# metaverse3d2022/Nerf-Cuda

Hardware: AMD Instinct MI355X
Metric: megasamples/s (march samples composited into a ray = the reference's per-ray sample count), Lego-like NeRF render @1920x1080 (higher is better)
Workload: dtype f16

## Files before the change

nerf-cuda_amd/csrc/nrf_api.hip:

```cpp

#include <hip/hip_runtime.h>

#include <chrono>
#include <cmath>
#include <cstdio>
#include <cstdlib>
#include <cstring>
#include <limits>
#include <mutex>
#include <string>
#include <vector>

#include "nrf_device.h"
#include "nrf_generic.h"
#include "nrf_launch.h"

using namespace nrf;

namespace {

thread_local std::string g_err;
int fail(int code, const std::string& msg) {
  g_err = msg;
  return code;
// ... 338 lines not shown
        const uint32_t res = Lv.res;
        Lv.q_off_b = far ? (uint32_t)(end_bytes >> 4) : (uint32_t)end_bytes;
        Lv.q_my_b = far ? res : res << 4;
        Lv.q_mz_b = far ? res * res : (res * res) << 4;
        Lv.q_max = res - 1;
        end_bytes += (uint64_t)res * res * (res + 1) * 16;
      }
    }
    p.table_bytes = end_bytes;
  }
  const uint32_t sh_b = F == 8 ? 4u : (F == 4 ? 3u : (F == 1 ? 1u : 2u));
  for (LevelParams& Lv : p.lp) {
    const bool hashed_pow2 = Lv.mode == LV_HASH_POW2;
    Lv.off_b = Lv.offset << sh_b;
    if (hashed_pow2) {
      Lv.my_b = 2654435761u << sh_b;
      Lv.mz_b = 805459861u << sh_b;
    } else {
      Lv.my_b = (Lv.my_b >> 2) << sh_b;
      Lv.mz_b = (Lv.mz_b >> 2) << sh_b;
    }
    Lv.mask_b = (hashed_pow2 || Lv.mode == LV_ADD_POW2) ? ((Lv.size - 1) << sh_b) : 0xffffffffu;
  }
  return p;
}

void nerf_matrix_to_ngp(const float p[16], float s, float R[9], float org[3]) {
  const int rows[3] = {1, 2, 0};
  for (int r = 0; r < 3; ++r) {
    const float* src = p + 4 * rows[r];
    R[3 * r + 0] = src[0];
    R[3 * r + 1] = -src[1];
    R[3 * r + 2] = -src[2];
    org[r] = src[3] * s + 0.0f;
  }
}

}

struct nrf_context {
  int device = 0;
  hipStream_t stream = nullptr;
  hipEvent_t ev0 = nullptr, ev1 = nullptr;
  bool model_loaded = false;
  nrf_model_desc desc{};
  nrf_level_table lv{};
  DevModel dm{};
  void* d_grid = nullptr;
  void* d_occ = nullptr;
  void* d_wfrag = nullptr;
  void* d_lv = nullptr;
  void* d_coarse = nullptr;
  void* d_dilated = nullptr;
  void* d_ctab = nullptr;
  void* d_gen = nullptr;
  void* d_wfrag_gen = nullptr;
  bool rays_persistent = false;
  int own_net = NET_HOT;
  void* d_wfrag_hot = nullptr;
  GenModel gen{};
  std::vector<float> host_grid;
  bool grid_missing = false;
  bool allow_persistent = true;
  bool centre_out = true;
  bool allow_gen_wlds = true;
  bool allow_width_instances = true;
  int queue_classes = 0;
  int n_cus = 256;
  nrf_options opt{};
  int W = 0, H = 0;
  int n_local_tiles = 0;
  int max_views = 1;
  int last_views = 1;
  size_t n_out_px = 0;
  size_t n_alloc_px = 0;
  void* d_rgba = nullptr;
  void* d_depth = nullptr;
  void* d_plan = nullptr;
  int plan_max_pos = 1 << 14;
  void* d_counters = nullptr;
  int call_index = 0;
  int quad_levels = -1;
  int quad_budget_mb = -1;
  uint64_t table_bytes = 0, table_ref_bytes = 0;
  uint32_t gather_addresses = 0;
  bool allow_gen_fast_grid = true;
  int march_ff = 1;
  int tail_split = 1;
  void* d_rgb8 = nullptr;
  void* d_depth8 = nullptr;
  void* bound_rgba = nullptr;
  void* bound_depth = nullptr;
  void* bound_rgbd8 = nullptr;
  void* bound_rgb8 = nullptr;
  void* bound_depth8 = nullptr;
  struct HostSlot {
    void* d_buf = nullptr;
    uint8_t* h_buf = nullptr;
    size_t views = 0, px = 0;
    hipEvent_t done = nullptr, t0 = nullptr, t1 = nullptr;
    hipEvent_t grp[2] = {nullptr, nullptr};
    std::vector<int> row_lo, row_hi;
    std::vector<int> col_lo, col_hi;
    int bg = -1;
    int n_views = 0, W = 0, H = 0;
    bool with_depth = true, pending = false;
    uint64_t copied = 0;
    std::vector<int> rows;
    unsigned* d_done = nullptr;
    unsigned* h_flags = nullptr;
    size_t prog_entries = 0;
    unsigned epoch = 0;
    bool progressive = false, copies_issued = false;
  } hs[2];
  int hs_next = 0;
  hipStream_t copy_stream = nullptr;
  bool host_merge = true;
  bool host_progressive = true;
  bool host_cols = true;
  bool host_skip_outside = true;
  void* last_rgba = nullptr;
  void* last_depth = nullptr;
  int march_budget = 256;
  bool sample_cap_forced = false;
  int sample_cap = 2;
  bool rendered = false;
  hipStream_t last_stream = nullptr;
};

namespace {

int set_device(nrf_context* c) {
  HIP_TRY(hipSetDevice(c->device));
  return NRF_OK;
}

void free_model(nrf_context* c) {
  if (c->d_grid) (void)hipFree(c->d_grid);
  if (c->d_occ) (void)hipFree(c->d_occ);
  if (c->d_wfrag) (void)hipFree(c->d_wfrag);
  if (c->d_lv) (void)hipFree(c->d_lv);
  if (c->d_coarse) (void)hipFree(c->d_coarse);
  if (c->d_ctab) (void)hipFree(c->d_ctab);
  if (c->d_dilated) (void)hipFree(c->d_dilated);
  if (c->d_gen) (void)hipFree(c->d_gen);
  if (c->d_wfrag_gen) (void)hipFree(c->d_wfrag_gen);
  if (c->d_wfrag_hot) (void)hipFree(c->d_wfrag_hot);
  c->d_wfrag_gen = c->d_wfrag_hot = nullptr;
  c->d_grid = c->d_occ = c->d_wfrag = c->d_lv = c->d_coarse = c->d_ctab = c->d_dilated = c->d_gen = nullptr;
  c->model_loaded = false;
}

constexpr int CALL_RING = 16;
constexpr size_t CALL_SLOT_BYTES = COUNTER_BYTES + 128 + 65536;
constexpr int HOST_SLOTS = 2;
constexpr uint32_t QUAD_BUDGET_MB_DEFAULT = 8192;
inline char* call_slot(const nrf_context* c, int index) { return (char*)c->d_counters + (size_t)(index % CALL_RING) * CALL_SLOT_BYTES; }

void free_host_slots(nrf_context* c) {
  for (auto& h : c->hs) {
    if (h.d_buf) (void)hipFree(h.d_buf);
    if (h.h_buf) (void)hipHostFree(h.h_buf);
    if (h.d_done) (void)hipFree(h.d_done);
    if (h.h_flags) (void)hipHostFree(h.h_flags);
    h.d_buf = nullptr;
    h.h_buf = nullptr;
    h.d_done = h.h_flags = nullptr;
    h.views = h.px = h.prog_entries = 0;
    h.bg = -1;
    h.pending = false;
  }
}

void free_frame(nrf_context* c) {
  if (c->d_rgba) (void)hipFree(c->d_rgba);
  if (c->d_depth) (void)hipFree(c->d_depth);
  if (c->d_rgb8) (void)hipFree(c->d_rgb8);
  if (c->d_depth8) (void)hipFree(c->d_depth8);
  c->d_rgba = c->d_depth = c->d_rgb8 = c->d_depth8 = nullptr;
  c->n_out_px = 0;
  c->rendered = false;
}

int total_strips(int W, int H) { return ((((W + 7) / 8) + 3) / 4) * ((H + 7) / 8); }

int local_tiles(int W, int H, int shard_index, int shard_count) {
  const int total = total_strips(W, H);
  if (shard_index >= total) return 0;
  return 4 * ((total - shard_index + shard_count - 1) / shard_count);
}

bool tiled_layout(const nrf_context* c) { return c->opt.shard_count > 1 || c->opt.tile_major != 0; }

int alloc_frame(nrf_context* c) {
  if (c->W <= 0 || c->H <= 0) return NRF_OK;
  const bool tiled = tiled_layout(c);
  c->n_local_tiles = local_tiles(c->W, c->H, c->opt.shard_index, c->opt.shard_count);
  int tps = 0;
  nrf_tiles_per_shard(c->W, c->H, c->opt.shard_count, &tps);
  const size_t per_view = tiled ? (size_t)tps * 64 : (size_t)c->W * c->H;
  const size_t need = per_view * (size_t)c->max_views;
  if (per_view == c->n_out_px && need == c->n_alloc_px && c->d_rgba) return NRF_OK;
  HIP_TRY(hipDeviceSynchronize());
  free_frame(c);
  HIP_TRY(hipMalloc(&c->d_rgba, need * 16));
  HIP_TRY(hipMalloc(&c->d_depth, need * 4));
  HIP_TRY(hipMemsetAsync(c->d_rgba, 0, need * 16, c->stream));
  HIP_TRY(hipMemsetAsync(c->d_depth, 0, need * 4, c->stream));
  HIP_TRY(hipStreamSynchronize(c->stream));
  c->n_out_px = per_view;
  c->n_alloc_px = need;
  return NRF_OK;
}

int fill_frame_params(nrf_context* c, const float cam[4], const float pose[16], FrameParams& P) {
  std::memset(&P, 0, sizeof(P));
  nerf_matrix_to_ngp(pose, c->desc.scale, P.R, P.org);
  for (int i = 0; i < 4; ++i) P.cam[i] = cam[i];
  P.W = c->W;
  P.H = c->H;
  P.tiles_x = (c->W + 7) / 8;
  P.tiles_y = (c->H + 7) / 8;
  P.shard_index = c->opt.shard_index;
  P.shard_count = c->opt.shard_count;
  P.n_local_tiles = c->n_local_tiles;
  P.tile_major = tiled_layout(c);
  P.bg_color = c->opt.bg_color;
  P.min_near = c->opt.min_near;
  P.dt_gamma = c->opt.dt_gamma;
  P.density_scale = c->opt.density_scale;
  P.max_steps = c->opt.max_steps;
  P.march_budget = c->march_budget;
  P.sample_cap = c->sample_cap;
  P.centre_out = c->centre_out ? 1 : 0;
  P.out_mode = c->bound_rgbd8 ? OUT_RGBD8 : (c->bound_rgb8 ? OUT_U8 : OUT_F32);
  P.skip_outside = 0;
  P.prog_done = P.prog_flags = nullptr;
  P.prog_epoch = 0;
  P.tail_split = c->tail_split;
  P.perturb = c->opt.perturb;
  P.march_ff = c->opt.perturb ? 0 : c->march_ff;
  P.fast_interp = c->opt.fast_interp ? 1 : 0;
  P.queue_classes = c->queue_classes;
  return NRF_OK;
}

void view_roi(const float R[9], const float org[3], const float cam[4], const float box[6], int W, int H, int roi[4]) {
  roi[0] = 0; roi[1] = 0; roi[2] = W - 1; roi[3] = H - 1;
  if (!(box[0] <= box[3])) {
    roi[2] = -1;
    roi[3] = -1;
    return;
  }
  const double a = R[0], b = R[1], cc = R[2], d = R[3], e = R[4], f = R[5], g = R[6], h = R[7], i = R[8];
  const double det = a * (e * i - f * h) - b * (d * i - f * g) + cc * (d * h - e * g);
  if (!(std::fabs(det) > 1e-12)) return;
  const double inv[9] = {(e * i - f * h) / det, (cc * h - b * i) / det, (b * f - cc * e) / det,
                         (f * g - d * i) / det, (a * i - cc * g) / det, (cc * d - a * f) / det,
                         (d * h - e * g) / det, (b * g - a * h) / det, (a * e - b * d) / det};
  double lo[2] = {1e300, 1e300}, hi[2] = {-1e300, -1e300};
  for (int c = 0; c < 8; ++c) {
    const double p[3] = {(double)box[(c & 1) ? 3 : 0] - org[0], (double)box[(c & 2) ? 4 : 1] - org[1],
                         (double)box[(c & 4) ? 5 : 2] - org[2]};
    const double vx = inv[0] * p[0] + inv[1] * p[1] + inv[2] * p[2];
    const double vy = inv[3] * p[0] + inv[4] * p[1] + inv[5] * p[2];
    const double vz = inv[6] * p[0] + inv[7] * p[1] + inv[8] * p[2];
    if (!(vz > 1e-3)) return;
    const double u = cam[2] + cam[0] * vx / vz, v = cam[3] + cam[1] * vy / vz;
    if (!(u == u) || !(v == v)) return;
    lo[0] = u < lo[0] ? u : lo[0]; hi[0] = u > hi[0] ? u : hi[0];
    lo[1] = v < lo[1] ? v : lo[1]; hi[1] = v > hi[1] ? v : hi[1];
  }
  const double m = 3.0;
  const double x0 = std::floor(lo[0] - 0.5 - m), y0 = std::floor(lo[1] - 0.5 - m);
  const double x1 = std::ceil(hi[0] - 0.5 + m), y1 = std::ceil(hi[1] - 0.5 + m);
  roi[0] = x0 < 0 ? 0 : (x0 > W ? W : (int)x0);
  roi[1] = y0 < 0 ? 0 : (y0 > H ? H : (int)y0);
  roi[2] = x1 < -1 ? -1 : (x1 > W - 1 ? W - 1 : (int)x1);
  roi[3] = y1 < -1 ? -1 : (y1 > H - 1 ? H - 1 : (int)y1);
}

int set_density_grid(nrf_context* c, const float* density_grid, float mean_density) {
  const nrf_model_desc* d = &c->desc;
  const uint64_t Hh = d->density_grid_size;
  const uint64_t cells = Hh * Hh * Hh * d->cascade;
  HIP_TRY(hipDeviceSynchronize());
  for (void** q : {&c->d_occ, &c->d_coarse, &c->d_ctab, &c->d_dilated}) {
    if (*q) (void)hipFree(*q);
    *q = nullptr;
  }
  const float thresh = fminf(0.01f, mean_density);
  std::vector<uint32_t> occ((cells + 31) / 32 + 1, 0u);
  for (uint64_t i = 0; i < cells; ++i)
    if (density_grid[i] > thresh) occ[i >> 5] |= 1u << (i & 31);

  const uint32_t Hs = d->density_grid_size, Cs = d->cascade;
  const uint32_t coarse_shift = (Hs % 4 == 0 && Hs >= 8) ? 2u : 0u;
  std::vector<uint32_t> coarse;
  if (coarse_shift) {
    const uint32_t Hc = Hs >> 2;
    coarse.assign(((uint64_t)Cs * Hc * Hc * Hc + 31) / 32 + 1, 0u);
    for (uint64_t i = 0; i < cells; ++i) {
      if (!((occ[i >> 5] >> (i & 31)) & 1u)) continue;
      const uint32_t level = (uint32_t)(i / (Hh * Hh * Hh));
      const uint64_t r = i % (Hh * Hh * Hh);
      const uint32_t nx = (uint32_t)(r / (Hh * Hh)), ny = (uint32_t)((r / Hh) % Hh), nz = (uint32_t)(r % Hh);
      const uint64_t cc = (((uint64_t)level * Hc + (nx >> 2)) * Hc + (ny >> 2)) * Hc + (nz >> 2);
      coarse[cc >> 5] |= 1u << (cc & 31);
    }
  }
  auto reachable = [&](uint32_t level, uint32_t nx, uint32_t ny, uint32_t nz) {
    if (level == 0 || Cs <= 1) return true;
    const double mb = fmin(ldexp(1.0, (int)level), (double)d->bound), cell = 2.0 * mb / (double)Hs;
    const uint32_t n3[3] = {nx, ny, nz};
    double r_max = 0.0;
    for (int a = 0; a < 3; ++a) {
      const double lo = -mb + n3[a] * cell, hi = lo + cell;
      r_max = fmax(r_max, fmax(fabs(lo), fabs(hi)));
    }
    return !(r_max + cell < ldexp(1.0, (int)level - 1));
  };
  float occ_box[6] = {1.f, 1.f, 1.f, -1.f, -1.f, -1.f};
  bool boundary_occupied = false;
  {
    bool any = false;
    for (uint32_t level = 0; level < Cs; ++level) {
      uint32_t lo[3] = {Hs, Hs, Hs}, hi[3] = {0, 0, 0};
      bool lvl_any = false;
      for (uint64_t r = 0; r < Hh * Hh * Hh; ++r) {
        const uint64_t i = (uint64_t)level * Hh * Hh * Hh + r;
        if (!((occ[i >> 5] >> (i & 31)) & 1u)) continue;
        const uint32_t n3[3] = {(uint32_t)(r / (Hh * Hh)), (uint32_t)((r / Hh) % Hh), (uint32_t)(r % Hh)};
        if (!reachable(level, n3[0], n3[1], n3[2])) continue;
        for (int a = 0; a < 3; ++a) { lo[a] = n3[a] < lo[a] ? n3[a] : lo[a]; hi[a] = n3[a] > hi[a] ? n3[a] : hi[a]; }
        lvl_any = true;
      }
      if (!lvl_any) continue;
      const double mip_bound = fmin(Cs > 1 ? ldexp(1.0, (int)level) : 1.0, (double)d->bound);
      const double cell = 2.0 * mip_bound / (double)Hs;
      for (int a = 0; a < 3; ++a) {
        float wlo = (float)(-mip_bound + ((double)lo[a] - 2.0) * cell);
        float whi = (float)(-mip_bound + ((double)hi[a] + 3.0) * cell);
        if (lo[a] == 0) wlo = fminf(wlo, fminf(d->aabb[a], -d->bound) - (float)(2.0 * cell));
        if (hi[a] == Hs - 1) whi = fmaxf(whi, fmaxf(d->aabb[a + 3], d->bound) + (float)(2.0 * cell));
        if (!any || wlo < occ_box[a]) occ_box[a] = wlo;
        if (!any || whi > occ_box[a + 3]) occ_box[a + 3] = whi;
        boundary_occupied = boundary_occupied || lo[a] == 0 || hi[a] == Hs - 1;
      }
      any = true;
    }
  }
  bool exterior_positions = false;
  {
    const float outer = fminf(Cs > 1 ? ldexpf(1.0f, (int)Cs - 1) : 1.0f, d->bound);
    exterior_positions = d->bound > outer;
    for (int a = 0; a < 3; ++a) exterior_positions = exterior_positions || d->aabb[a] < -d->bound || d->aabb[a + 3] > d->bound;
  }
  const bool visibility_walk = !(exterior_positions && boundary_occupied);
  std::vector<uint32_t> dilated;
  uint32_t dilated_level_words = 0;
  if (coarse_shift && visibility_walk) {
    const int Hc = (int)(Hs >> 2), Hf = (int)Hs;
    dilated_level_words = (uint32_t)(((uint64_t)Hc * Hc * Hc + 31) / 32);
    dilated.assign((size_t)dilated_level_words * Cs, 0u);
    for (uint32_t level = 0; level < Cs; ++level) {
      uint32_t* dl = dilated.data() + (size_t)level * dilated_level_words;
      for (int x = 0; x < Hf; ++x)
        for (int y = 0; y < Hf; ++y)
          for (int z = 0; z < Hf; ++z) {
            const uint64_t i = (((uint64_t)level * Hf + x) * Hf + y) * Hf + z;
            if (!((occ[i >> 5] >> (i & 31)) & 1u)) continue;
            if (!reachable(level, (uint32_t)x, (uint32_t)y, (uint32_t)z)) continue;
            for (int dx = -1; dx <= 1; ++dx)
              for (int dy = -1; dy <= 1; ++dy)
                for (int dz = -1; dz <= 1; ++dz) {
                  const int X = x + dx, Y = y + dy, Z = z + dz;
                  if (X < 0 || Y < 0 || Z < 0 || X >= Hf || Y >= Hf || Z >= Hf) continue;
                  const uint64_t nn = ((uint64_t)(X >> 2) * Hc + (Y >> 2)) * Hc + (Z >> 2);
                  dl[nn >> 5] |= 1u << (nn & 31);
                }
          }
    }
  }
  std::vector<float> ctab((size_t)Cs * (Hs + 1));
  for (uint32_t level = 0; level < Cs; ++level) {
    const float mip_bound = fminf(Cs > 1 ? ldexpf(1.0f, (int)level) : 1.0f, d->bound);
    const float Hm1 = (float)(Hs - 1);
    for (uint32_t v = 0; v <= Hs; ++v) ctab[(size_t)level * (Hs + 1) + v] = ((float)v / Hm1 * 2 - 1) * mip_bound;
  }

  auto upload = [&](void** dst, const void* src, size_t bytes) -> hipError_t {
    hipError_t e = hipMalloc(dst, bytes);
    if (e != hipSuccess) return e;
    return hipMemcpyAsync(*dst, src, bytes, hipMemcpyHostToDevice, c->stream);
  };
  HIP_TRY(upload(&c->d_occ, occ.data(), occ.size() * 4));
  if (coarse_shift) HIP_TRY(upload(&c->d_coarse, coarse.data(), coarse.size() * 4));
  HIP_TRY(upload(&c->d_ctab, ctab.data(), ctab.size() * 4));
  if (!dilated.empty()) HIP_TRY(upload(&c->d_dilated, dilated.data(), dilated.size() * 4));
  HIP_TRY(hipStreamSynchronize(c->stream));
  HIP_TRY(hipDeviceSynchronize());
  DevModel& M = c->dm;
  M.occ_bits = (const uint32_t*)c->d_occ;
  for (int i = 0; i < 6; ++i) M.occ_box[i] = occ_box[i];
  M.occ_coarse = (const uint32_t*)c->d_coarse;
  M.cell_bound = (const float*)c->d_ctab;
  M.occ_dilated = (const uint32_t*)c->d_dilated;
  M.coarse_shift = coarse_shift;
  M.lds_coarse_words = M.lds_ctab_floats = M.lds_dilated_words = 0;
  {
    const uint64_t words = coarse_shift ? (uint64_t)coarse.size() : 0, fl = ctab.size();
    uint64_t budget = (uint64_t)render_lds_table_max_bytes();
    if (M.stage == NET_GENERIC) {
      const uint64_t used = (uint64_t)render_gen_lds_fixed_bytes(M.gen_wave_bytes);
      budget = used + budget <= 160u * 1024u ? budget : 160u * 1024u - used;
    }
    if (M.stage == NET_WIDE) {
      const uint64_t room = 160u * 1024u / 3u - (uint64_t)render_wide_lds_fixed_bytes();
      budget = budget < room ? budget : room;
    }
    if (coarse_shift && 4 * (words + fl) <= budget) {
      M.lds_coarse_words = (uint32_t)words;
      M.lds_ctab_floats = (uint32_t)fl;
    }
  }
  M.dilated_level_words = dilated_level_words;
  if (!dilated.empty() && dilated.size() * 4 <= (size_t)N_FRAGS * 64 * 16) M.lds_dilated_words = (uint32_t)dilated.size();
  M.net = M.stage;
  M.persistent = 0;
  M.persist_waves = 0;
  M.gen_weights_lds = 0;
  M.n_cus = (uint32_t)c->n_cus;
  if (c->allow_persistent && M.lds_coarse_words > 0) {
    const size_t tables = 4 * ((size_t)M.lds_coarse_words + M.lds_ctab_floats + dilated.size());
    const int form = march_form(M.H, M.cascade, M.bound);
    for (const int net : {c->own_net, (int)M.stage}) {
      const int first_waves = render_persist_waves(net, form);
      for (int waves : {first_waves, net == NET_GENERIC && first_waves != 8 ? 8 : 0}) {
        if (waves == 0 || M.persistent) break;
        const size_t fixed = (size_t)render_persistent_lds_bytes(net, waves, M.gen_wave_bytes) + tables;
        for (int wlds : {1, 0}) {
          if (wlds && (net != NET_GENERIC || !c->allow_gen_wlds)) continue;
          if (fixed + (wlds ? 16u + M.gen_frag_bytes : 0u) <= 160u * 1024u) {
            M.net = (uint32_t)net;
            M.persistent = 1;
            M.persist_waves = (uint32_t)waves;
            M.gen_weights_lds = (uint32_t)wlds;
            M.lds_dilated_words = (uint32_t)dilated.size();
            break;
          }
        }
      }
      if (M.persistent) break;
    }
  }
  c->rays_persistent = M.persistent != 0 && M.net == NET_HOT;
  c->desc.mean_density = mean_density;
  c->host_grid.assign(density_grid, density_grid + cells);
  return NRF_OK;
}
// ... 48 lines not shown

int nrf_tiles_per_shard(int width, int height, int shard_count, int* n) {
  if (!n || width <= 0 || height <= 0 || shard_count <= 0) return fail(NRF_E_INVALID, "bad argument");
  *n = 4 * ((total_strips(width, height) + shard_count - 1) / shard_count);
  return NRF_OK;
}

int nrf_create(int device, nrf_context** out) {
  if (!out) return fail(NRF_E_INVALID, "null argument");
  int count = 0;
  hipError_t e = hipGetDeviceCount(&count);
  if (e != hipSuccess || count <= 0)
    return fail(NRF_E_NODEVICE, "no HIP device available (this library has no CPU fallback)");
  if (device < 0 || device >= count) return fail(NRF_E_NODEVICE, "device index out of range");
  hipDeviceProp_t prop;
  HIP_TRY(hipGetDeviceProperties(&prop, device));
  if (std::strncmp(prop.gcnArchName, "gfx950", 6) != 0)
    return fail(NRF_E_NODEVICE, std::string("device is ") + prop.gcnArchName + ", this library is built for gfx950 only");
  nrf_context* c = new nrf_context;
  c->device = device;
  nrf_default_options(&c->opt);
  if (const char* e = std::getenv("NRF_MARCH_BUDGET")) {
    const int b = std::atoi(e);
    if (b >= 1 && b <= 4096) c->march_budget = b;
  }
  if (const char* e = std::getenv("NRF_SAMPLE_CAP")) { c->sample_cap = std::atoi(e); c->sample_cap_forced = true; }
  if (const char* e = std::getenv("NRF_PERSISTENT")) c->allow_persistent = std::atoi(e) != 0;
  if (const char* e = std::getenv("NRF_CENTRE_OUT")) c->centre_out = std::atoi(e) != 0;
  if (const char* e = std::getenv("NRF_GEN_WLDS")) c->allow_gen_wlds = std::atoi(e) != 0;
  if (const char* e = std::getenv("NRF_WIDTH_INSTANCES")) c->allow_width_instances = std::atoi(e) != 0;
  if (const char* e = std::getenv("NRF_QUEUE_CLASSES")) c->queue_classes = std::atoi(e);
  c->n_cus = prop.multiProcessorCount > 0 ? prop.multiProcessorCount : 256;
  HIP_TRY(hipSetDevice(device));
  HIP_TRY(hipStreamCreateWithFlags(&c->stream, hipStreamNonBlocking));
  HIP_TRY(hipEventCreate(&c->ev0));
  HIP_TRY(hipEventCreate(&c->ev1));
  if (const char* e = std::getenv("NRF_HOST_PROGRESSIVE")) c->host_progressive = std::atoi(e) != 0;
  if (const char* e = std::getenv("NRF_HOST_MERGE")) c->host_merge = std::atoi(e) != 0;
  if (const char* e = std::getenv("NRF_HOST_SKIP_OUTSIDE")) c->host_skip_outside = std::atoi(e) != 0;
  if (const char* e = std::getenv("NRF_HOST_COLS")) c->host_cols = std::atoi(e) != 0;
  {
    int prio_lo = 0, prio_hi = 0;
    HIP_TRY(hipDeviceGetStreamPriorityRange(&prio_lo, &prio_hi));
    HIP_TRY(hipStreamCreateWithPriority(&c->copy_stream, hipStreamNonBlocking, prio_hi));
  }
  for (auto& h : c->hs) {
    HIP_TRY(hipEventCreateWithFlags(&h.done, hipEventDisableTiming));
    for (hipEvent_t& g : h.grp) HIP_TRY(hipEventCreateWithFlags(&g, hipEventDisableTiming));
    HIP_TRY(hipEventCreate(&h.t0));
    HIP_TRY(hipEventCreate(&h.t1));
  }
  if (const char* e = std::getenv("NRF_TAIL_SPLIT")) c->tail_split = std::atoi(e) != 0 ? 1 : 0;
  if (const char* e = std::getenv("NRF_MARCH_FF")) c->march_ff = std::atoi(e) != 0 ? 1 : 0;
  if (const char* e = std::getenv("NRF_GEN_FAST_GRID")) c->allow_gen_fast_grid = std::atoi(e) != 0;
  if (const char* e = std::getenv("NRF_QUAD_LEVELS")) c->quad_levels = std::atoi(e);
  if (const char* e = std::getenv("NRF_QUAD_BUDGET_MB")) c->quad_budget_mb = std::max(0, std::atoi(e));
  HIP_TRY(hipMalloc(&c->d_counters, CALL_RING * CALL_SLOT_BYTES));
  HIP_TRY(hipMemset(c->d_counters, 0, CALL_RING * CALL_SLOT_BYTES));
  if (const char* e = std::getenv("NRF_PLAN_MAX_POS")) c->plan_max_pos = std::max(0, std::min(std::atoi(e), (int)PLAN_CAP));
  HIP_TRY(hipMalloc(&c->d_plan, CALL_RING * PLAN_BYTES));
  HIP_TRY(hipMemset(c->d_plan, 0, CALL_RING * PLAN_BYTES));
  *out = c;
  return NRF_OK;
}

int nrf_destroy(nrf_context* c) {
  if (!c) return NRF_OK;
  (void)hipSetDevice(c->device);
  (void)hipDeviceSynchronize();
  free_model(c);
  free_frame(c);
  free_host_slots(c);
  for (auto& h : c->hs) {
    if (h.done) (void)hipEventDestroy(h.done);
    for (hipEvent_t g : h.grp) if (g) (void)hipEventDestroy(g);
    if (h.t0) (void)hipEventDestroy(h.t0);
    if (h.t1) (void)hipEventDestroy(h.t1);
  }
  if (c->copy_stream) (void)hipStreamDestroy(c->copy_stream);
  if (c->d_counters) (void)hipFree(c->d_counters);
  if (c->d_plan) (void)hipFree(c->d_plan);
  if (c->ev0) (void)hipEventDestroy(c->ev0);
  if (c->ev1) (void)hipEventDestroy(c->ev1);
  if (c->stream) (void)hipStreamDestroy(c->stream);
  delete c;
  return NRF_OK;
}

int nrf_load_model(nrf_context* c, const nrf_model_desc* d) {
  if (!c || !d || !d->params) return fail(NRF_E_INVALID, "null argument");
  if (d->abi_version != NRF_ABI_VERSION) return fail(NRF_E_INVALID, "abi_version mismatch");
  int rc = set_device(c);
  if (rc) return rc;
  {
    nrf_level_table lv;
    rc = validate_model(*d, lv);
    if (rc) return rc;
  }
  HIP_TRY(hipDeviceSynchronize());
  free_model(c);
  uint64_t budget_mb = QUAD_BUDGET_MB_DEFAULT;
  {
    size_t mem_free = 0, mem_total = 0;
    if (hipMemGetInfo(&mem_free, &mem_total) == hipSuccess) budget_mb = std::min<uint64_t>((uint64_t)mem_total >> 24, (uint64_t)mem_free >> 21);
    else (void)hipGetLastError();
  }
// ... 712 lines not shown
}

int nrf_render_batch(nrf_context* c, int n_views, const float* cams, const float* poses, void* stream, nrf_frame* out) {
  return nrf_render_views(c, n_views, cams, poses, stream, out);
}

int nrf_render(nrf_context* c, const float cam[4], const float pose[16], void* stream, nrf_frame* out) {
  if (!cam || !pose) return fail(NRF_E_INVALID, "null argument");
  return nrf_render_views(c, 1, cam, pose, stream, out);
}

int nrf_debug_counters(nrf_context* c, unsigned long long out[16]) {
  if (!c || !out) return fail(NRF_E_INVALID, "null argument");
  HIP_TRY(hipEventSynchronize(c->ev1));
  unsigned long long raw[COUNTER_SLOTS * 16];
  HIP_TRY(hipMemcpy(raw, call_slot(c, c->call_index), COUNTER_BYTES, hipMemcpyDeviceToHost));
  for (int i = 0; i < 16; ++i) {
    out[i] = 0;
    for (int sl = 0; sl < COUNTER_SLOTS; ++sl) out[i] = i == 14 ? std::max(out[i], raw[sl * 16 + i]) : out[i] + raw[sl * 16 + i];
  }
  return NRF_OK;
}

extern "C" int nrf_debug_instance(nrf_context* c) {
  if (!c || !c->model_loaded) return -1;
  const int net = (int)c->dm.net;
  const int code = net == NET_HOT ? 0 : net == NET_GENERIC ? 1 : net == NET_WIDE ? 2 : net == NET_WIDE_SH ? 4 : net_grid_f(net) ? 5 : 3;
  return code + (c->dm.persistent ? 16 : 0);
}

extern "C" int nrf_debug_rays_instance(nrf_context* c) {
  if (!c || !c->model_loaded) return -1;
  if (c->rays_persistent) return 16;
  const int st = (int)c->dm.stage;
  return st == NET_GENERIC ? 1 : st == NET_WIDE ? 2 : 0;
}

extern "C" int nrf_debug_ray_valid(const float o[3], const float d[3]) {
  if (!o || !d) return 0;
  return ray_valid(o, d) ? 1 : 0;
}

extern "C" int nrf_debug_plan(const nrf_model_desc* d, int allow_own, uint64_t budget_mb, uint32_t out[6]) {
  if (!d || !d->params || !out) return fail(NRF_E_INVALID, "null argument");
  const ModelPlan p = plan_model(*d, allow_own != 0, budget_mb, 4);
  if (p.rc) return p.rc;
  const int waves = render_persist_waves(p.own, march_form(d->density_grid_size, d->cascade, d->bound));
  const uint32_t v[6] = {(uint32_t)p.own, (uint32_t)p.stage, p.quad_mask, p.quad_far, (uint32_t)waves,
                         (uint32_t)render_persistent_lds_bytes(p.own, waves, p.gen_wave_bytes)};
  std::memcpy(out, v, sizeof(v));
  return NRF_OK;
}

extern "C" int nrf_debug_wave_times(nrf_context* c, unsigned long long* out, int n_waves) {
  if (!c || !out || n_waves < 1 || n_waves > 4096) return fail(NRF_E_INVALID, "bad argument");
  HIP_TRY(hipEventSynchronize(c->ev1));
  HIP_TRY(hipMemcpy(out, call_slot(c, c->call_index) + COUNTER_BYTES + 128, (size_t)n_waves * 16, hipMemcpyDeviceToHost));
  return NRF_OK;
}

int nrf_render_async(nrf_context* c, const float cam[4], const float pose[16], nrf_frame* out) {
  if (!c) return fail(NRF_E_INVALID, "null context");
  return nrf_render(c, cam, pose, (void*)c->stream, out);
}

int nrf_sync(nrf_context* c) {
  if (!c) return fail(NRF_E_INVALID, "null context");
  int rc = set_device(c);
  if (rc) return rc;
  HIP_TRY(hipStreamSynchronize(c->stream));
  if (c->last_stream && c->last_stream != c->stream) HIP_TRY(hipStreamSynchronize(c->last_stream));
  return NRF_OK;
}

int nrf_bind_output(nrf_context* c, void* rgba, void* depth) {
  if (!c) return fail(NRF_E_INVALID, "null context");
  if ((rgba == nullptr) != (depth == nullptr)) return fail(NRF_E_INVALID, "bind both planes or neither");
  c->bound_rgba = rgba;
  c->bound_depth = depth;
  c->bound_rgbd8 = nullptr;
  c->bound_rgb8 = c->bound_depth8 = nullptr;
  return NRF_OK;
}

int nrf_bind_output_rgbd8(nrf_context* c, void* rgbd8) {
  if (!c) return fail(NRF_E_INVALID, "null context");
  c->bound_rgbd8 = rgbd8;
  if (rgbd8) c->bound_rgba = c->bound_depth = c->bound_rgb8 = c->bound_depth8 = nullptr;
  return NRF_OK;
}

int nrf_bind_output_u8(nrf_context* c, void* rgb8, void* depth8) {
  if (!c) return fail(NRF_E_INVALID, "null context");
  if ((rgb8 == nullptr) != (depth8 == nullptr)) return fail(NRF_E_INVALID, "bind both planes or neither");
  if (((uintptr_t)rgb8 | (uintptr_t)depth8) & 3u) return fail(NRF_E_INVALID, "8-bit planes must be 4-byte aligned");
  c->bound_rgb8 = rgb8;
  c->bound_depth8 = depth8;
  if (rgb8) c->bound_rgba = c->bound_depth = c->bound_rgbd8 = nullptr;
  return NRF_OK;
}

int nrf_get_stats(nrf_context* c, nrf_stats* s) {
  if (!c || !s) return fail(NRF_E_INVALID, "null argument");
  if (!c->rendered) return fail(NRF_E_STATE, "nothing rendered yet");
  int rc = set_device(c);
  if (rc) return rc;
// ... 252 lines not shown
```

nerf-cuda_amd/csrc/nrf_device.h:

```cpp
#pragma once

#include <hip/hip_runtime.h>
#include <stdint.h>

#include "../../include/nerfhip.h"

namespace nrf {

typedef _Float16 half_t;
typedef _Float16 half2_t __attribute__((ext_vector_type(2)));
typedef _Float16 half4_t __attribute__((ext_vector_type(4)));
typedef _Float16 half8_t __attribute__((ext_vector_type(8)));
typedef float float2_t __attribute__((ext_vector_type(2)));
typedef float float4_t __attribute__((ext_vector_type(4)));

enum : uint32_t {
  LV_DENSE = 0,
  LV_HASH_POW2 = 1,
  LV_GENERIC = 2,
  LV_ADD_POW2 = 3
};

struct LevelParams {
  float scale;
// ... 26 lines not shown
  FRAG_R0X = 24,
  N_FRAGS_WIDE_ALL = 32
};
constexpr int RK_WIDE = 3;
template <int W>
struct MlpShape {
  static_assert(W == 16 || W == 32 || W == 64 || W == 128, "FullyFusedMLP widths");
  static constexpr int MT = W / 16, KS = (W + 31) / 32;
  static constexpr int D0 = 0, D1 = MT, R0 = MT + KS, R1 = 2 * MT + KS, R2 = 2 * MT + KS + MT * KS, N = 2 * MT + 2 * KS + MT * KS;
};
static_assert(MlpShape<64>::D1 == FRAG_D1 && MlpShape<64>::R0 == FRAG_R0 && MlpShape<64>::R1 == FRAG_R1 && MlpShape<64>::R2 == FRAG_R2 &&
                  MlpShape<64>::N == N_FRAGS, "MlpShape<64> is the base.json layout");

enum : int { DF_D0 = 0, DF_D1 = 4, DF_R0 = 6, DF_R2 = 10, DF_WW = 12, DEPTH_MAX_WW = 5, DEPTH_FRAGS = DF_WW + 8 * DEPTH_MAX_WW };

struct DevModel {
  const uint32_t* grid;
  const uint32_t* occ_bits;
  const uint32_t* occ_coarse;
  const float* cell_bound;
  uint32_t grid_bytes;
  const uint32_t* occ_dilated;
  uint32_t dilated_level_words;
  uint32_t pos_w_pow2;
  const uint4* wfrag;
  const LevelParams* lv;
  float aabb[6];
  float occ_box[6];
  float bound;
  float rbound;
  float pos_w;
  uint32_t cascade;
  uint32_t H;
  uint32_t n_levels;
  uint32_t dir_encoding, sh_degree, n_frequencies;
  uint32_t density_activation, density_output_activation, sigma_activation;
  uint32_t rgb_activation, rgb_output_activation;
  uint32_t uni_modes;
  uint32_t net;
  uint32_t stage;
  const struct GenModel* gen;
  uint32_t gen_wave_bytes;
  uint32_t coarse_shift;
  uint32_t lds_coarse_words;
  uint32_t lds_ctab_floats;
  uint32_t lds_dilated_words;
  uint32_t persistent;
  uint32_t persist_waves;
  uint32_t gen_frag_bytes;
  uint32_t gen_weights_lds;
  uint32_t n_cus;
  uint32_t depth_xd, depth_xr;
  const uint4* wfrag_hot;
  uint32_t grid_smooth;
  uint32_t grid_nearest;
  uint32_t dir_w;
  uint32_t quad_far;
  uint32_t quad_mask;
};

struct ViewParams {
  float R[9];
  float org[3];
  float cam[4];
  int roi[4];
  int k_lo, k_hi, q_begin, q_rows, q_row0;
};
constexpr int COUNTER_SLOTS = 64;
constexpr int COUNTER_BYTES = COUNTER_SLOTS * 16 * 8;
constexpr int MAX_VIEWS = 128;
struct ViewBatch {
  ViewParams v[MAX_VIEWS];
  int n_views;
  int blocks_per_view;
  int q_total;
  int n_classes, class_cols;
  unsigned long long view_stride_px;
};

enum : int { OUT_F32 = 0, OUT_RGBD8 = 1, OUT_U8 = 2 };
struct FrameParams {
  float R[9];
  float org[3];
  float cam[4];
  int W, H;
  int tiles_x, tiles_y;
  int shard_index, shard_count;
  int n_local_tiles;
  int tile_major;
  float bg_color, min_near, dt_gamma, density_scale;
  int max_steps;
  int march_budget;
  int queue_classes;
  int out_mode;
  int skip_outside;
  int centre_out;
  int prog_epoch;
  int fast_interp;
  int tail_split;
  int march_ff;
  int perturb;
  int sample_cap;
  unsigned* prog_done;
  unsigned* prog_flags;
  const unsigned* plan_order;
  const float* rays_o;
  const float* rays_d;
  unsigned rays_per_view;
};

constexpr float MAX_CAMERA_DISTANCE = 4096.0f;
constexpr float RAY_DIR_NORM2_MIN = 0.25f, RAY_DIR_NORM2_MAX = 4.0f;
__host__ __device__ inline bool ray_valid(const float o[3], const float d[3]) {
  const float o2 = o[0] * o[0] + (o[1] * o[1] + o[2] * o[2]);
  const float d2 = d[0] * d[0] + (d[1] * d[1] + d[2] * d[2]);
  return o2 <= MAX_CAMERA_DISTANCE * MAX_CAMERA_DISTANCE && d2 >= RAY_DIR_NORM2_MIN && d2 <= RAY_DIR_NORM2_MAX;
}

__device__ __forceinline__ float clampf(float x, float lo, float hi) { return fminf(hi, fmaxf(lo, x)); }
__device__ __forceinline__ uint32_t h2_bits(half2_t v) { return __builtin_bit_cast(uint32_t, v); }
__device__ __forceinline__ half2_t bits_h2(uint32_t v) { return __builtin_bit_cast(half2_t, v); }
__device__ __forceinline__ uint32_t pack_h2(float a, float b) {
  half2_t v;
  v.x = (half_t)a;
  v.y = (half_t)b;
  return h2_bits(v);
}
__device__ __forceinline__ int lane_id() { return (int)(threadIdx.x & 63u); }
__device__ __forceinline__ half_t f2h_rne(float v) {
  asm("" : "+v"(v));
  return (half_t)v;
}

__device__ __forceinline__ float activate(uint32_t act, float v) {
  switch (act) {
    case NRF_ACT_RELU: return v > 0.0f ? v : 0.0f;
    case NRF_ACT_EXPONENTIAL: return expf(v);
    case NRF_ACT_SIGMOID: return 1.0f / (1.0f + expf(-v));
    case NRF_ACT_SQUAREPLUS: {
      const float x = v * 10.0f;
      return 0.5f * (x + sqrtf(x * x + 4)) / 10.0f;
    }
    case NRF_ACT_SOFTPLUS: return logf(expf(v * 10.0f) + 1.0f) / 10.0f;
    case NRF_ACT_SINE: return sinf(v);
    default: return v;
  }
}

__device__ __forceinline__ float activate_native(uint32_t act, float v) {
  switch (act) {
    case NRF_ACT_RELU: return fmaxf(v, 0.0f);
    case NRF_ACT_EXPONENTIAL: return __expf(v);
    case NRF_ACT_SIGMOID: return __builtin_amdgcn_rcpf(1.0f + __expf(-v));
// ... 94 lines not shown

struct MarchConst {
  float bound, rbound, dt_gamma, dt_min, dt_max, Hf, Hm1;
  uint32_t H, C, HH, HHH;
  uint32_t coarse_shift;
  uint32_t Hc;
  uint32_t log2H;
  float halfH;
  int log2_bound;
};

__device__ __forceinline__ MarchConst march_const(const DevModel& M, float dt_gamma) {
  MarchConst c;
  c.bound = M.bound;
  c.rbound = M.rbound;
  c.dt_gamma = dt_gamma;
  c.dt_min = 2 * 1.7320508075688772f / 1024;
  c.dt_max = 2 * M.bound / (float)M.H;
  c.H = M.H;
  c.C = M.cascade;
  c.HH = M.H * M.H;
  c.HHH = M.H * M.H * M.H;
  c.Hf = (float)M.H;
  c.Hm1 = (float)(M.H - 1);
  c.coarse_shift = M.coarse_shift;
  c.Hc = M.H >> M.coarse_shift;
  c.log2H = 31u - (uint32_t)__builtin_clz(M.H | 1u);
  c.halfH = 0.5f * (float)M.H;
  {
    int e;
    (void)frexpf(M.bound, &e);
    c.log2_bound = e - 1;
  }
  return c;
}

__device__ __forceinline__ float pcg32_first_float(uint64_t initstate, uint64_t initseq) {
  const uint64_t MULT = 0x5851f42d4c957f2dULL;
  const uint64_t inc = (initseq << 1u) | 1u;
  uint64_t state = inc;
  state += initstate;
  state = state * MULT + inc;
  const uint32_t xorshifted = (uint32_t)(((state >> 18u) ^ state) >> 27u);
  const uint32_t rot = (uint32_t)(state >> 59u);
  const uint32_t r = (xorshifted >> rot) | (xorshifted << ((~rot + 1u) & 31u));
  return __builtin_bit_cast(float, (r >> 9) | 0x3f800000u) - 1.0f;
}

enum : int { MARCH_FOUND = 0, MARCH_EXHAUSTED = 1, MARCH_OUT_OF_BUDGET = 2 };

__device__ __forceinline__ float clamp3(float x, float lo, float hi) { return __builtin_amdgcn_fmed3f(x, lo, hi); }

enum : int { MARCH_GENERIC = 0, MARCH_UNIT = 1, MARCH_POW2 = 2 };
template <bool COARSE, int MODE>
__device__ __forceinline__ int march_next(const MarchConst& c, const uint32_t* __restrict__ occ, const uint32_t* coarse,
                                          const float* ctab, float ox, float oy, float oz, float dx, float dy, float dz,
                                          float rdx, float rdy, float rdz, int sx, int sy, int sz, float far, float t_skip,
                                          int& budget, float& t, float& x, float& y, float& z, float& dt_out) {
  while (t < far) {
    if (budget <= 0) return MARCH_OUT_OF_BUDGET;
    --budget;
#ifdef NRF_DIAG_EXTRA_MARCH
#pragma unroll
    for (int e = 0; e < NRF_DIAG_EXTRA_MARCH; ++e) {
      float sink;
      asm volatile("v_mul_f32 %0, %1, %2" : "=v"(sink) : "v"(t), "v"(dx));
    }
#endif
#ifdef NRF_DIAG_FF_UPPER
    if (t < t_skip) {
      do {
        t += clamp3(t * c.dt_gamma, c.dt_min, c.dt_max);
      } while (t < t_skip && t < far);
      continue;
    }
#endif
    x = clamp3(ox + t * dx, -c.bound, c.bound);
    y = clamp3(oy + t * dy, -c.bound, c.bound);
    z = clamp3(oz + t * dz, -c.bound, c.bound);
    constexpr bool UNIT = MODE == MARCH_UNIT, POW2 = MODE == MARCH_POW2;
    int level = 0;
    int nx, ny, nz;
    if (UNIT) {
      nx = (int)clamp3(__builtin_fmaf(x, c.halfH, c.halfH), 0.0f, c.Hm1);
      ny = (int)clamp3(__builtin_fmaf(y, c.halfH, c.halfH), 0.0f, c.Hm1);
      nz = (int)clamp3(__builtin_fmaf(z, c.halfH, c.halfH), 0.0f, c.Hm1);
    } else if (POW2) {
      const float mx = fmaxf(fabsf(x), fmaxf(fabsf(y), fabsf(z)));
      int exponent;
      (void)frexpf(mx, &exponent);
      level = min(max(exponent, 0), (int)c.C - 1);
      const float scale = ldexpf(c.halfH, -min(level, c.log2_bound));
      nx = (int)clamp3(__builtin_fmaf(x, scale, c.halfH), 0.0f, c.Hm1);
      ny = (int)clamp3(__builtin_fmaf(y, scale, c.halfH), 0.0f, c.Hm1);
      nz = (int)clamp3(__builtin_fmaf(z, scale, c.halfH), 0.0f, c.Hm1);
    } else {
      float mip_bound = fminf(1.0f, c.bound), mip_rbound;
      if (c.C > 1) {
        const float mx = fmaxf(fabsf(x), fmaxf(fabsf(y), fabsf(z)));
        int exponent;
        (void)frexpf(mx, &exponent);
        level = (int)fminf((float)c.C - 1, fmaxf(0.0f, (float)exponent));
        mip_bound = fminf(ldexpf(1.0f, level), c.bound);
      }
      mip_rbound = (mip_bound == c.bound) ? c.rbound : ldexpf(1.0f, -level);
      nx = (int)clamp3((0.5f * (x * mip_rbound + 1)) * c.Hf, 0.0f, c.Hm1);
      ny = (int)clamp3((0.5f * (y * mip_rbound + 1)) * c.Hf, 0.0f, c.Hm1);
      nz = (int)clamp3((0.5f * (z * mip_rbound + 1)) * c.Hf, 0.0f, c.Hm1);
    }
    const uint32_t cell = (UNIT || POW2) ? ((((((uint32_t)level << c.log2H) | (uint32_t)nx) << c.log2H) | (uint32_t)ny) << c.log2H) | (uint32_t)nz
                                         : (uint32_t)level * c.HHH + (uint32_t)nx * c.HH + (uint32_t)ny * c.H + (uint32_t)nz;
    const float* tab = UNIT ? ctab : ctab + (uint32_t)level * (c.H + 1);
    const float bx = tab[nx + sx], by = tab[ny + sy], bz = tab[nz + sz];
    bool occupied = false;
    if (!(t < t_skip)) {
      if (COARSE) {
        const uint32_t lc = c.log2H - 2u;
        const uint32_t cc = (UNIT || POW2) ? (((((((uint32_t)level << lc) | ((uint32_t)nx >> 2)) << lc) | ((uint32_t)ny >> 2)) << lc) | ((uint32_t)nz >> 2))
                                           : ((uint32_t)level * c.Hc + ((uint32_t)nx >> 2)) * c.Hc * c.Hc + ((uint32_t)ny >> 2) * c.Hc + ((uint32_t)nz >> 2);
        const bool coarse_occ = (coarse[cc >> 5] >> (cc & 31u)) & 1u;
        if (coarse_occ) occupied = (occ[cell >> 5] >> (cell & 31u)) & 1u;
      } else {
        occupied = (occ[cell >> 5] >> (cell & 31u)) & 1u;
      }
    }
    if (occupied) {
      dt_out = clamp3(t * c.dt_gamma, c.dt_min, c.dt_max);
      return MARCH_FOUND;
    }
    const float tx = (bx - x) * rdx;
    const float ty = (by - y) * rdy;
    const float tz = (bz - z) * rdz;
    const float tt = t + fmaxf(0.0f, fminf(tx, fminf(ty, tz)));
    do {
      t += clamp3(t * c.dt_gamma, c.dt_min, c.dt_max);
    } while (t < tt);
  }
  return MARCH_EXHAUSTED;
}

#ifndef NRF_MARCH_FF
#define NRF_MARCH_FF 1
#endif
__device__ __forceinline__ float barrier_before(const float* ctab, int H, float mb, float mag, float o, float d, float rd, float t_skip) {
  const float NONE = -3.402823466e+38f;
  if (!(d < 0.0f) || !(rd > -3.0e38f)) return NONE;
  const float xs = o + t_skip * d;
  const float v = clamp3(ceilf((xs / mb + 1.0f) * (0.5f * (float)(H - 1))), 0.0f, (float)H);
  int n = (int)v;
  if (n > H - 1) return NONE;
  const float eps = 4.0e-6f * mag * (1.0f + fabsf(rd));
  float e = (ctab[n] - o) * rd + eps;
  if (!(e <= t_skip)) {
    if (++n > H - 1) return NONE;
    e = (ctab[n] - o) * rd + eps;
  }
  return e <= t_skip ? e : NONE;
}

__device__ __forceinline__ float fast_forward_to_barrier(const MarchConst& c, const float* ctab, float mb, const float o[3], const float d[3],
                                                         float rdx, float rdy, float rdz, float t, float t_skip, float far) {
  const float mag = t_skip + c.bound + 2.0f;
  const float tb = fminf(fmaxf(barrier_before(ctab, (int)c.H, mb, mag, o[0], d[0], rdx, t_skip),
                               fmaxf(barrier_before(ctab, (int)c.H, mb, mag, o[1], d[1], rdy, t_skip),
                                     barrier_before(ctab, (int)c.H, mb, mag, o[2], d[2], rdz, t_skip))), far);
  while (t < tb) t += clamp3(t * c.dt_gamma, c.dt_min, c.dt_max);
  return t;
}

__device__ __forceinline__ bool cube_interval(float s, const float o[3], const float rd[3], float& t_in, float& t_out) {
  bool ok = true;
  t_in = -3.402823466e+38f;
  t_out = 3.402823466e+38f;
#pragma unroll
// ... 686 lines not shown
```

nerf-cuda_amd/csrc/nrf_render.h:

```cpp

#pragma once
#include <cstddef>
#include <cstdlib>

#include "nrf_device.h"
#include "nrf_generic.h"
#include "nrf_launch.h"

namespace nrf {

#ifndef NRF_SLOTS
#define NRF_SLOTS 64
#endif
constexpr int SLOTS = NRF_SLOTS;
struct WaveLds {
  union {
    float4 pos[SLOTS];
    float4 out[SLOTS];
  };
  float2 aux[SLOTS];
  uint32_t dirf[64][8];
};
static_assert(sizeof(WaveLds) == 2048 + 24 * SLOTS, "WaveLds layout");

// ... 565 lines not shown
          if (old & (1u << hw)) {
            const int rank = (int)__builtin_amdgcn_mbcnt_hi((unsigned)(alive_mask >> 32), __builtin_amdgcn_mbcnt_lo((unsigned)alive_mask, 0u));
            const bool give = alive && (rank & 1);
            const unsigned long long gm = __ballot(give);
            const int slot = (int)__builtin_amdgcn_mbcnt_hi((unsigned)(gm >> 32), __builtin_amdgcn_mbcnt_lo((unsigned)gm, 0u));
            uint32_t* mb = reinterpret_cast<uint32_t*>(reinterpret_cast<WaveLds*>(ha->wave_blocks) + hw);
            if (give) {
              auto put = [&](int f, float v) { mb[f * 32 + slot] = __builtin_bit_cast(uint32_t, v); };
              mb[HELP_PIX * 32 + slot] = pix_idx;
              put(HELP_D0, d[0]); put(HELP_D1, d[1]); put(HELP_D2, d[2]);
              put(HELP_NEAR, near); put(HELP_FAR, far); put(HELP_FAR_M, far_m);
              put(HELP_T, t); put(HELP_TC, tc);
              put(HELP_WS, ws); put(HELP_DEP, dep); put(HELP_CR, cr); put(HELP_CG, cg); put(HELP_CB, cb);
              mb[HELP_NSAMP * 32 + slot] = (uint32_t)n_ray_samples;
            }
            if (lane == 0) {
              __hip_atomic_fetch_add(&hl->busy, 1, __ATOMIC_RELAXED, __HIP_MEMORY_SCOPE_WORKGROUP);
              __hip_atomic_store(&hl->mail[hw], 0x80000000u | ((unsigned)ha->view << 8) | (unsigned)__popcll(gm), __ATOMIC_RELEASE,
                                 __HIP_MEMORY_SCOPE_WORKGROUP);
            }
            alive = alive && !give;
            given = given || give;
          }
        }
      }
    }
    NRF_STAMP(t0);
    unsigned long long slots = 0ull;
    int cnt = 0, S = 0;
    int budget = P.march_budget;
    bool marching = alive;
    bool ended = false;
    float o[3] = {o_in[0], o_in[1], o_in[2]};
    if constexpr (RAYS) {
      o[0] = o[1] = o[2] = 0.f;
      if (alive) {
        uint32_t pi = pix_idx;
        asm volatile("" : "+v"(pi));
        const uint32_t off = 3u * ray_number(P, pi);
        const float* ov = P.rays_o + 3 * (size_t)rays_view * P.rays_per_view;
        o[0] = ov[off];
        o[1] = ov[off + 1u];
        o[2] = ov[off + 2u];
      }
    }
    const float Tq = 1.0f - ws;
    int cap = 8;
    if (P.sample_cap == 1) cap = Tq < 0.02f ? 1 : (Tq < 0.1f ? 2 : (Tq < 0.4f ? 4 : 8));
    else if (P.sample_cap == 2) {
      int e;
      (void)__builtin_frexpf(Tq, &e);
      cap = min(max(e + 13, 1), 8);
    }
    for (int k = 0; k < 8; ++k) {
      const unsigned long long mm = __ballot(marching);
      if (mm == 0ull || S + __popcll(mm) > SLOTS) break;
      float x = 0.f, y = 0.f, z = 0.f, dt = 0.f;
      bool found = false;
#ifdef NRF_PHASE_TIMING
      const int budget_before = budget;
#endif
      float last_t = tc;
      if constexpr (PERTURB) {
        last_t = tc + mc.dt_min * pcg32_first_float((uint64_t)ray_number(P, pix_idx), (uint64_t)(uint32_t)P.perturb);
        if (t == tc) t = last_t;
      }
      if (marching) {
        const int r = COARSE_LDS ? march_next<true, MARCH>(mc, M.occ_bits, coarse_lds, ctab_lds, o[0], o[1], o[2], d[0], d[1], d[2], rdx,
                                                    rdy, rdz, sx, sy, sz, far_m, t_skip, budget, t, x, y, z, dt)
                                 : march_next<false, MARCH_GENERIC>(mc, M.occ_bits, nullptr, M.cell_bound, o[0], o[1], o[2], d[0], d[1], d[2], rdx,
                                                     rdy, rdz, sx, sy, sz, far_m, t_skip, budget, t, x, y, z, dt);
        found = r == MARCH_FOUND;
        marching = found;
        ended = ended || r == MARCH_EXHAUSTED;
      }
#ifdef NRF_PHASE_TIMING
      {
        int used = budget_before - budget;
        n_lane_trips += (unsigned)used;
        for (int o = 32; o; o >>= 1) used = max(used, __shfl_xor(used, o));
        n_wave_iters += (unsigned)used;
      }
#endif
      const unsigned long long fm = __ballot(found);
      if (found) {
        const int slot = S + (int)__builtin_amdgcn_mbcnt_hi((unsigned)(fm >> 32), __builtin_amdgcn_mbcnt_lo((unsigned)fm, 0u));
        const float tn = t + dt;
        const float delta = tn - last_t;
        tc = tc + delta;
        t = tc;
        W->pos[slot] = make_float4(x, y, z, __builtin_bit_cast(float, lane));
        W->aux[slot] = make_float2(dt, tc);
        slots |= (unsigned long long)slot << (8 * k);
        cnt++;
        if (n_ray_samples + cnt >= P.max_steps) { marching = false; ended = true; }
        else if (cnt >= cap) marching = false;
      }
      S += __popcll(fm);
    }
    wave_sync();
    NRF_STAMP(t1);

    if (S > 0) {
      network_dispatch<NET, FAST>(M, wl, lvs, W, lm.gen, S, lane, P.density_scale);
      wave_sync();
    }
    NRF_STAMP(t2);

    if (alive) {
      bool terminated = false;
      for (int k = 0; k < 8; ++k) {
        if (k >= cnt) break;
        const int slot = (int)((slots >> (8 * k)) & 0xffull);
        const float4 so = W->out[slot];
        const float2 dtc = W->aux[slot];
        const float alpha = 1.0f - __expf(-so.w * dtc.x);
        const float T = 1 - ws;
        const float wgt = alpha * T;
        ws += wgt;
        dep += wgt * dtc.y;
        cr += wgt * so.x;
        cg += wgt * so.y;
// ... 765 lines not shown
```

Before: 14840.

## Add 4x4x4 occupancy bricks with per-ray brick cache in march

```diff
diff --git a/nerf-cuda_amd/csrc/nrf_api.hip b/nerf-cuda_amd/csrc/nrf_api.hip
--- a/nerf-cuda_amd/csrc/nrf_api.hip
+++ b/nerf-cuda_amd/csrc/nrf_api.hip
@@ -414,6 +414,7 @@
   void* d_lv = nullptr;
   void* d_coarse = nullptr;
   void* d_dilated = nullptr;
+  void* d_bricks = nullptr;
   void* d_ctab = nullptr;
   void* d_gen = nullptr;
   void* d_wfrag_gen = nullptr;
@@ -449,6 +450,7 @@
   bool allow_gen_fast_grid = true;
   int march_ff = 1;
   int tail_split = 1;
+  int occ_bricks = 1;
   void* d_rgb8 = nullptr;
   void* d_depth8 = nullptr;
   void* bound_rgba = nullptr;
@@ -505,11 +507,12 @@
   if (c->d_coarse) (void)hipFree(c->d_coarse);
   if (c->d_ctab) (void)hipFree(c->d_ctab);
   if (c->d_dilated) (void)hipFree(c->d_dilated);
+  if (c->d_bricks) (void)hipFree(c->d_bricks);
   if (c->d_gen) (void)hipFree(c->d_gen);
   if (c->d_wfrag_gen) (void)hipFree(c->d_wfrag_gen);
   if (c->d_wfrag_hot) (void)hipFree(c->d_wfrag_hot);
   c->d_wfrag_gen = c->d_wfrag_hot = nullptr;
-  c->d_grid = c->d_occ = c->d_wfrag = c->d_lv = c->d_coarse = c->d_ctab = c->d_dilated = c->d_gen = nullptr;
+  c->d_grid = c->d_occ = c->d_wfrag = c->d_lv = c->d_coarse = c->d_ctab = c->d_dilated = c->d_bricks = c->d_gen = nullptr;
   c->model_loaded = false;
 }
 
@@ -601,6 +604,7 @@
   P.prog_epoch = 0;
   P.tail_split = c->tail_split;
   P.perturb = c->opt.perturb;
+  P.occ_bricks = c->occ_bricks;
   P.march_ff = c->opt.perturb ? 0 : c->march_ff;
   P.fast_interp = c->opt.fast_interp ? 1 : 0;
   P.queue_classes = c->queue_classes;
@@ -642,12 +646,39 @@
   roi[3] = y1 < -1 ? -1 : (y1 > H - 1 ? H - 1 : (int)y1);
 }
 
+void pack_occ_coarse(const uint32_t* occ, uint32_t C, uint32_t H, uint32_t* out) {
+  const uint64_t Hc = H >> 2, Hh = H, cells = (uint64_t)C * Hh * Hh * Hh;
+  for (uint64_t i = 0; i < cells; ++i) {
+    if (!((occ[i >> 5] >> (i & 31)) & 1u)) continue;
+    const uint32_t level = (uint32_t)(i / (Hh * Hh * Hh));
+    const uint64_t r = i % (Hh * Hh * Hh);
+    const uint32_t nx = (uint32_t)(r / (Hh * Hh)), ny = (uint32_t)((r / Hh) % Hh), nz = (uint32_t)(r % Hh);
+    const uint64_t cc = (((uint64_t)level * Hc + (nx >> 2)) * Hc + (ny >> 2)) * Hc + (nz >> 2);
+    out[cc >> 5] |= 1u << (cc & 31);
+  }
+}
+
+void pack_occ_bricks(const uint32_t* occ, uint32_t C, uint32_t H, uint64_t* out) {
+  const uint64_t Hc = H >> 2, Hh = H;
+  for (uint64_t i = 0; i < (uint64_t)C * Hc * Hc * Hc; ++i) out[i] = 0ull;
+  for (uint64_t level = 0; level < C; ++level)
+    for (uint64_t nx = 0; nx < Hh; ++nx)
+      for (uint64_t ny = 0; ny < Hh; ++ny)
+        for (uint64_t nz = 0; nz < Hh; nz += 4) {
+          const uint64_t i = ((level * Hh + nx) * Hh + ny) * Hh + nz;
+          const uint64_t row = (occ[i >> 5] >> (i & 31)) & 0xfull;
+          if (!row) continue;
+          const uint64_t cc = ((level * Hc + (nx >> 2)) * Hc + (ny >> 2)) * Hc + (nz >> 2);
+          out[cc] |= row << (((nx & 3) << 4) | ((ny & 3) << 2));
+        }
+}
+
 int set_density_grid(nrf_context* c, const float* density_grid, float mean_density) {
   const nrf_model_desc* d = &c->desc;
   const uint64_t Hh = d->density_grid_size;
   const uint64_t cells = Hh * Hh * Hh * d->cascade;
   HIP_TRY(hipDeviceSynchronize());
-  for (void** q : {&c->d_occ, &c->d_coarse, &c->d_ctab, &c->d_dilated}) {
+  for (void** q : {&c->d_occ, &c->d_coarse, &c->d_ctab, &c->d_dilated, &c->d_bricks}) {
     if (*q) (void)hipFree(*q);
     *q = nullptr;
   }
@@ -662,14 +693,7 @@
   if (coarse_shift) {
     const uint32_t Hc = Hs >> 2;
     coarse.assign(((uint64_t)Cs * Hc * Hc * Hc + 31) / 32 + 1, 0u);
-    for (uint64_t i = 0; i < cells; ++i) {
-      if (!((occ[i >> 5] >> (i & 31)) & 1u)) continue;
-      const uint32_t level = (uint32_t)(i / (Hh * Hh * Hh));
-      const uint64_t r = i % (Hh * Hh * Hh);
-      const uint32_t nx = (uint32_t)(r / (Hh * Hh)), ny = (uint32_t)((r / Hh) % Hh), nz = (uint32_t)(r % Hh);
-      const uint64_t cc = (((uint64_t)level * Hc + (nx >> 2)) * Hc + (ny >> 2)) * Hc + (nz >> 2);
-      coarse[cc >> 5] |= 1u << (cc & 31);
-    }
+    pack_occ_coarse(occ.data(), Cs, Hs, coarse.data());
   }
   auto reachable = [&](uint32_t level, uint32_t nx, uint32_t ny, uint32_t nz) {
     if (level == 0 || Cs <= 1) return true;
@@ -758,6 +782,12 @@
   };
   HIP_TRY(upload(&c->d_occ, occ.data(), occ.size() * 4));
   if (coarse_shift) HIP_TRY(upload(&c->d_coarse, coarse.data(), coarse.size() * 4));
+  std::vector<uint64_t> bricks;
+  if (coarse_shift) {
+    bricks.resize((size_t)Cs * (Hs >> 2) * (Hs >> 2) * (Hs >> 2));
+    pack_occ_bricks(occ.data(), Cs, Hs, bricks.data());
+    HIP_TRY(upload(&c->d_bricks, bricks.data(), bricks.size() * 8));
+  }
   HIP_TRY(upload(&c->d_ctab, ctab.data(), ctab.size() * 4));
   if (!dilated.empty()) HIP_TRY(upload(&c->d_dilated, dilated.data(), dilated.size() * 4));
   HIP_TRY(hipStreamSynchronize(c->stream));
@@ -768,6 +798,7 @@
   M.occ_coarse = (const uint32_t*)c->d_coarse;
   M.cell_bound = (const float*)c->d_ctab;
   M.occ_dilated = (const uint32_t*)c->d_dilated;
+  M.occ_bricks = (const uint64_t*)c->d_bricks;
   M.coarse_shift = coarse_shift;
   M.lds_coarse_words = M.lds_ctab_floats = M.lds_dilated_words = 0;
   {
@@ -922,6 +953,7 @@
   }
   if (const char* e = std::getenv("NRF_TAIL_SPLIT")) c->tail_split = std::atoi(e) != 0 ? 1 : 0;
   if (const char* e = std::getenv("NRF_MARCH_FF")) c->march_ff = std::atoi(e) != 0 ? 1 : 0;
+  if (const char* e = std::getenv("NRF_OCC_BRICKS")) c->occ_bricks = std::atoi(e) != 0 ? 1 : 0;
   if (const char* e = std::getenv("NRF_GEN_FAST_GRID")) c->allow_gen_fast_grid = std::atoi(e) != 0;
   if (const char* e = std::getenv("NRF_QUAD_LEVELS")) c->quad_levels = std::atoi(e);
   if (const char* e = std::getenv("NRF_QUAD_BUDGET_MB")) c->quad_budget_mb = std::max(0, std::atoi(e));
@@ -1740,6 +1772,19 @@
   return NRF_OK;
 }
 
+extern "C" int nrf_debug_pack_occ_bricks(const uint32_t* occ, uint32_t C, uint32_t H, uint64_t* out) {
+  if (!occ || !out || C == 0 || H < 8 || H % 4 != 0) return fail(NRF_E_INVALID, "bad argument");
+  pack_occ_bricks(occ, C, H, out);
+  return NRF_OK;
+}
+extern "C" int nrf_debug_pack_occ_coarse(const uint32_t* occ, uint32_t C, uint32_t H, uint32_t* out) {
+  if (!occ || !out || C == 0 || H < 8 || H % 4 != 0) return fail(NRF_E_INVALID, "bad argument");
+  const uint64_t Hc = H >> 2, words = ((uint64_t)C * Hc * Hc * Hc + 31) / 32;
+  for (uint64_t i = 0; i < words; ++i) out[i] = 0u;
+  pack_occ_coarse(occ, C, H, out);
+  return NRF_OK;
+}
+
 extern "C" int nrf_debug_wave_times(nrf_context* c, unsigned long long* out, int n_waves) {
   if (!c || !out || n_waves < 1 || n_waves > 4096) return fail(NRF_E_INVALID, "bad argument");
   HIP_TRY(hipEventSynchronize(c->ev1));
diff --git a/nerf-cuda_amd/csrc/nrf_device.h b/nerf-cuda_amd/csrc/nrf_device.h
--- a/nerf-cuda_amd/csrc/nrf_device.h
+++ b/nerf-cuda_amd/csrc/nrf_device.h
@@ -102,6 +102,7 @@
   uint32_t n_cus;
   uint32_t depth_xd, depth_xr;
   const uint4* wfrag_hot;
+  const uint64_t* occ_bricks;
   uint32_t grid_smooth;
   uint32_t grid_nearest;
   uint32_t dir_w;
@@ -149,6 +150,7 @@
   int fast_interp;
   int tail_split;
   int march_ff;
+  int occ_bricks;
   int perturb;
   int sample_cap;
   unsigned* prog_done;
@@ -349,11 +351,17 @@
 __device__ __forceinline__ float clamp3(float x, float lo, float hi) { return __builtin_amdgcn_fmed3f(x, lo, hi); }
 
 enum : int { MARCH_GENERIC = 0, MARCH_UNIT = 1, MARCH_POW2 = 2 };
+struct BrickCache {
+  const uint64_t* bricks;
+  uint32_t tag;
+  uint64_t bits;
+};
 template <bool COARSE, int MODE>
 __device__ __forceinline__ int march_next(const MarchConst& c, const uint32_t* __restrict__ occ, const uint32_t* coarse,
                                           const float* ctab, float ox, float oy, float oz, float dx, float dy, float dz,
                                           float rdx, float rdy, float rdz, int sx, int sy, int sz, float far, float t_skip,
-                                          int& budget, float& t, float& x, float& y, float& z, float& dt_out) {
+                                          int& budget, float& t, float& x, float& y, float& z, float& dt_out,
+                                          BrickCache* bc = nullptr) {
   while (t < far) {
     if (budget <= 0) return MARCH_OUT_OF_BUDGET;
     --budget;
@@ -415,8 +423,21 @@
         const uint32_t lc = c.log2H - 2u;
         const uint32_t cc = (UNIT || POW2) ? (((((((uint32_t)level << lc) | ((uint32_t)nx >> 2)) << lc) | ((uint32_t)ny >> 2)) << lc) | ((uint32_t)nz >> 2))
                                            : ((uint32_t)level * c.Hc + ((uint32_t)nx >> 2)) * c.Hc * c.Hc + ((uint32_t)ny >> 2) * c.Hc + ((uint32_t)nz >> 2);
-        const bool coarse_occ = (coarse[cc >> 5] >> (cc & 31u)) & 1u;
-        if (coarse_occ) occupied = (occ[cell >> 5] >> (cell & 31u)) & 1u;
+#ifdef NRF_DIAG_OCC_UPPER
+        occupied = (coarse[cc >> 5] >> (cc & 31u)) & 1u;
+#else
+        if (bc != nullptr && bc->bricks != nullptr) {
+          if (cc != bc->tag) {
+            bc->tag = cc;
+            bc->bits = 0ull;
+            if ((coarse[cc >> 5] >> (cc & 31u)) & 1u) bc->bits = bc->bricks[cc];
+          }
+          occupied = (bc->bits >> ((((uint32_t)nx & 3u) << 4) | (((uint32_t)ny & 3u) << 2) | ((uint32_t)nz & 3u))) & 1ull;
+        } else {
+          const bool coarse_occ = (coarse[cc >> 5] >> (cc & 31u)) & 1u;
+          if (coarse_occ) occupied = (occ[cell >> 5] >> (cell & 31u)) & 1u;
+        }
+#endif
       } else {
         occupied = (occ[cell >> 5] >> (cell & 31u)) & 1u;
       }
diff --git a/nerf-cuda_amd/csrc/nrf_render.h b/nerf-cuda_amd/csrc/nrf_render.h
--- a/nerf-cuda_amd/csrc/nrf_render.h
+++ b/nerf-cuda_amd/csrc/nrf_render.h
@@ -641,6 +641,8 @@
       (void)__builtin_frexpf(Tq, &e);
       cap = min(max(e + 13, 1), 8);
     }
+    constexpr bool BRICKS = COARSE_LDS && !(NET == NET_WIDE && HELP);
+    BrickCache brick = {(BRICKS && P.occ_bricks != 0) ? M.occ_bricks : nullptr, ~0u, 0ull};
     for (int k = 0; k < 8; ++k) {
       const unsigned long long mm = __ballot(marching);
       if (mm == 0ull || S + __popcll(mm) > SLOTS) break;
@@ -656,7 +658,7 @@
       }
       if (marching) {
         const int r = COARSE_LDS ? march_next<true, MARCH>(mc, M.occ_bits, coarse_lds, ctab_lds, o[0], o[1], o[2], d[0], d[1], d[2], rdx,
-                                                    rdy, rdz, sx, sy, sz, far_m, t_skip, budget, t, x, y, z, dt)
+                                                    rdy, rdz, sx, sy, sz, far_m, t_skip, budget, t, x, y, z, dt, BRICKS ? &brick : nullptr)
                                  : march_next<false, MARCH_GENERIC>(mc, M.occ_bits, nullptr, M.cell_bound, o[0], o[1], o[2], d[0], d[1], d[2], rdx,
                                                      rdy, rdz, sx, sy, sz, far_m, t_skip, budget, t, x, y, z, dt);
         found = r == MARCH_FOUND;
```

Result: no change. 14820 (-0.2%).
